# iastro-pt/gpyrn

Hardware: AMD Instinct MI355X
Metric: ELBO iterations/sec (N=4096, P=3, Q=2) (higher is better)
Workload: dtype f64; 1 GPU; BASELINE config 3: N=4096, p=3 outputs, q=2 nodes, QP nodes / SE weights, synthetic RV series (seed 0); latent_gps=8, comm_ranks=1

## Files before the change

### gpyrn_amd/_hip.py

```python
import ctypes
import os
from ctypes import POINTER, byref, c_char, c_char_p, c_double, c_int, c_int32, c_int64, c_void_p

import numpy as np

_HERE = os.path.dirname(os.path.abspath(__file__))
LIB_PATH = os.environ.get('GPRN_HIP_LIB') or os.path.join(_HERE, 'libgprn_hip.so')

GPRN_E_ARG, GPRN_E_HIP, GPRN_E_NODEV, GPRN_E_COMM, GPRN_E_NOMEM, GPRN_E_UNSUPPORTED = -1, -2, -3, -4, -5, -6
GPRN_BATCH_FORCED = 1
COV_JOINT = 1
ORDER_REFERENCE, ORDER_SEQUENTIAL = 0, 1
ELBO_REFERENCE, ELBO_BOUND = 0, 1
M_K, M_KLINV, M_SIGMA, M_BX, M_BL = 0, 1, 2, 3, 4
T_NAMES = ('fill', 'build_B', 'diag', 'panel', 'update', 'lauum', 'vec', 'update_ahead')
TILE = 128

_dp = POINTER(c_double)


class BackendUnavailable(RuntimeError):
    """libgprn_hip.so is not built, or there is no MI355X to run it on."""


# ... 13 lines not shown
    'gprn_comm_unique_id': (c_int, [POINTER(c_char)]),
    'gprn_comm_init': (c_int, [c_void_p, c_int, c_int, POINTER(c_char)]),
    'gprn_set_owners': (c_int, [c_void_p, POINTER(c_int)]),
    'gprn_comm_barrier_max': (c_int, [c_void_p, _dp]),
    'gprn_set_kernel': (c_int, [c_void_p, c_int, POINTER(c_int32), c_int, _dp, c_int, c_int]),
    'gprn_upload_K': (c_int, [c_void_p, c_int, _dp]),
    'gprn_set_y_resid': (c_int, [c_void_p, _dp]),
    'gprn_set_jitters': (c_int, [c_void_p, _dp]),
    'gprn_factor_priors': (c_int, [c_void_p]),
    'gprn_set_muvar': (c_int, [c_void_p, _dp, _dp]),
    'gprn_get_muvar': (c_int, [c_void_p, _dp, _dp]),
    'gprn_sweep': (c_int, [c_void_p, c_int, c_int, _dp, _dp]),
    'gprn_predict': (c_int, [c_void_p, c_int, _dp, _dp, _dp]),
    'gprn_predict_upload': (c_int, [c_void_p, c_int, c_int, _dp, _dp, _dp]),
    'gprn_predict_cov': (c_int, [c_void_p, c_int, _dp, c_int, _dp, _dp, _dp]),
    'gprn_predict_draws': (c_int, [c_void_p, c_int, _dp, c_int, _dp, _dp, _dp, _dp]),
    'gprn_predict_upload_kss': (c_int, [c_void_p, c_int, c_int, _dp]),
    'gprn_get_scalars': (c_int, [c_void_p, _dp]),
    'gprn_keep_sigma': (c_int, [c_void_p, c_int]),
    'gprn_get_matrix': (c_int, [c_void_p, c_int, c_int, _dp]),
    'gprn_get_logdet_K': (c_int, [c_void_p, _dp]),
    'gprn_profile_enable': (c_int, [c_void_p, c_int]),
    'gprn_profile_read': (c_int, [c_void_p, _dp, POINTER(c_int64), c_int]),
    'gprn_test_gemm': (c_int, [c_void_p, c_int, c_int, c_int, c_int, c_int, c_int, _dp, _dp, _dp]),
    'gprn_comm_allreduce_sum': (c_int, [c_void_p, _dp, c_int]),
    'gprn_test_factor_invert': (c_int, [c_void_p, c_int, c_int, _dp, _dp, _dp]),
    'gprn_test_lauum': (c_int, [c_void_p, c_int, _dp, _dp]),
    'gprn_test_gemm_rate': (c_int, [c_void_p, c_int, c_int, c_int, c_int, c_int, _dp]),
    'gprn_test_fill_rate': (c_int, [c_void_p, c_int, _dp]),
    'gprn_test_mfma_peak': (c_int, [c_void_p, c_int, c_int, _dp]),
    'gprn_test_tile_launch': (c_int, [c_void_p, c_int, c_int, _dp, c_int, POINTER(c_int64), c_int, c_int, c_int, _dp, c_int,
                              c_int]),
    'gprn_test_tile_step': (c_int, [c_void_p, c_int, _dp, c_int, c_int, c_int, c_int, POINTER(c_int64)]),
    'gprn_set_option': (c_int, [c_void_p, c_char_p, c_int, POINTER(c_int)]),
    'gprn_elbocalc_batch': (c_int, [c_void_p, c_int, _dp, c_int, _dp, _dp, _dp, _dp, c_int, _dp, POINTER(c_int), POINTER(c_int),
                            POINTER(c_int), _dp, _dp]),
    'gprn_elbocalc_batch_grad': (c_int, [c_void_p, c_int, _dp, c_int, _dp, _dp, _dp, _dp, c_int, c_int, _dp, POINTER(c_int),
                                 POINTER(c_int), POINTER(c_int), _dp, _dp, _dp]),
    'gprn_predict_batch': (c_int, [c_void_p, c_int, _dp, c_int, _dp, _dp, _dp, c_int, _dp, _dp, _dp, _dp, _dp, POINTER(c_int)]),
    'gprn_test_predict_fill': (c_int, [c_void_p, c_int, c_int, _dp, c_int, _dp, c_int, c_int, c_int, _dp, _dp, _dp, _dp]),
    'gprn_elbocalc': (c_int, [c_void_p, c_int, _dp, _dp, _dp, _dp, c_int, _dp, c_int, POINTER(c_int), POINTER(c_int),
                      POINTER(c_int), _dp, _dp]),
    'gprn_expected_loglike': (c_int, [c_void_p, _dp]),
    'gprn_prior_terms': (c_int, [c_void_p, c_int, _dp, _dp, _dp]),
    'gprn_grad_matrices': (c_int, [c_void_p, c_int, _dp, _dp]),
    'gprn_grad_kernel': (c_int, [c_void_p, c_int, _dp, _dp]),
    'gprn_grad_elbo': (c_int, [c_void_p, _dp, c_int]),
    'gprn_grad_matrix': (c_int, [c_void_p, c_int, _dp]),
    'gprn_eval_kernel': (c_int, [c_void_p, POINTER(c_int32), c_int, _dp, c_int, c_double, _dp]),
    'gprn_eval_kernel_grad': (c_int, [c_void_p, POINTER(c_int32), c_int, _dp, c_int, _dp]),
    'gprn_sample_prior': (c_int, [c_void_p, POINTER(c_int32), c_int, _dp, c_int, c_double, c_int, _dp, _dp]),
}

_lib = None


def load_library():
    global _lib
    if _lib is not None:
        return _lib
    if not os.path.exists(LIB_PATH):
        raise BackendUnavailable(
            f'{LIB_PATH} is missing: build it with `python -c "import __graft_entry__ as g; '
            f'g.build()"` (or make -C gpyrn_amd/csrc)')
    try:
        lib = ctypes.CDLL(LIB_PATH)
# ... 357 lines not shown
            raise ValueError('tstar is empty')
        jt = None
        if outputs:
            if jitters is None:
                raise ValueError('predict_batch: the output pair needs the jitters')
            jt = _f64(jitters)
            if jt.size != B * self.p:
                raise ValueError(f'jitters must be (B, p) = ({B}, {self.p}), got {jt.shape}')
        ns = ts.size
        lm = np.empty((B, self.G, ns)) if latent else None
        lv = np.empty((B, self.G, ns)) if latent else None
        om = np.empty((B, self.p, ns)) if outputs else None
        ov = np.empty((B, self.p, ns)) if outputs else None
        info = np.zeros(B, dtype=np.int32)
        opt = lambda a: None if a is None else _ptr(a)
        rc = self._lib.gprn_predict_batch(self._h, B, _ptr(kp), kp.shape[1], _ptr(m0), _ptr(v0), opt(jt), ns, _ptr(ts),
                                          opt(lm), opt(lv), opt(om), opt(ov), info.ctypes.data_as(POINTER(c_int)))
        if rc == GPRN_E_UNSUPPORTED:
            return None
        self._check(rc, 'predict_batch')
        return lm, lv, om, ov, info.astype(int)

    def test_predict_fill(self, kernel_params, var, eval_index, gp, tstar, batched):
        kp = _f64(np.atleast_2d(kernel_params))
        B = kp.shape[0]
        v0 = _f64(np.reshape(var, (B, (self.p + 1) * self.q * self.N)))
        ts = _f64(np.ravel(tstar))
        K, Ks, kss = np.empty((self.N, self.N)), np.empty((ts.size, self.N)), np.empty(ts.size)
        self._check(self._lib.gprn_test_predict_fill(self._h, int(bool(batched)), B, _ptr(kp), kp.shape[1], _ptr(v0),
                                                     int(eval_index), int(gp), ts.size, _ptr(ts), _ptr(K), _ptr(Ks), _ptr(kss)),
                    'test_predict_fill')
        return K, Ks, kss

    def option(self, name, value=-1):
        old = c_int(0)
        self._check(self._lib.gprn_set_option(self._h, name.encode(), int(value), byref(old)), 'set_option')
        return old.value

    def profile_enable(self, families=T_NAMES):
        mask = 0
        for f in families or ():
            mask |= 1 << T_NAMES.index(f)
        self._check(self._lib.gprn_profile_enable(self._h, mask), 'profile_enable')

    def profile_read(self, reset=True):
        ms = np.zeros(len(T_NAMES))
        n = np.zeros(len(T_NAMES), dtype=np.int64)
        self._check(self._lib.gprn_profile_read(self._h, _ptr(ms), n.ctypes.data_as(POINTER(c_int64)),
                                                int(bool(reset))), 'profile_read')
        return {k: (float(ms[i]), int(n[i])) for i, k in enumerate(T_NAMES)}

    def test_gemm(self, A, B, C, a_mode, b_mode, c_mode):
        A, B = _f64(A), _f64(B)
        C = _f64(C).copy()
        M, K = A.shape
        K2, N = B.shape
        assert K == K2 and C.shape == (M, N)
        self._check(self._lib.gprn_test_gemm(self._h, M, N, K, a_mode, b_mode, c_mode,
                                             _ptr(A), _ptr(B), _ptr(C)), 'test_gemm')
        return C

    def test_factor_invert(self, A):
        A = _f64(A)
        if A.ndim == 2:
            A = A[None]
        batch, n, _ = A.shape
# ... 49 lines not shown
```

### gpyrn_amd/csrc/api_sweep.hip

```cpp
#include "api_internal.h"

static int factor_priors_impl(gprn_ctx* c);

extern "C" int gprn_factor_priors(gprn_ctx* c)
{
    DeviceLock lock_(c);
    WatchScope watch_(c, "gprn_factor_priors");
    if (!c || !c->N) return bad(c, "factor_priors: call set_data first");
    HIP_TRY(c, hipSetDevice(c->device));
    if (c->owner.empty()) return bad(c, "factor_priors: call set_owners first");
    c->grad_ready = false;
    int pre = GPRN_OK;
    for (int g = 0; g < c->G && !pre; ++g)
        if (!c->kspec[g].set) pre = bad(c, "factor_priors: a latent GP has no kernel");
    if ((pre = agree_to_start(c, pre, "factor_priors"))) return pre;
    return with_event_fallback(c, "factor_priors", [&](bool) { return factor_priors_impl(c); }, true);
}

static int ensure_small_sweep_tabs(gprn_ctx* c)
{
    if (c->small_sweep_ready) return GPRN_OK;
    std::vector<double*> ktab(c->q, nullptr);
    for (int j = 1; j < c->q && c->elbo_form == GPRN_ELBO_REFERENCE; ++j) {
        if (!c->Kinv[j]) return bad(c, "small path: K_j^-1 of a node is missing (no set-up yet?)");
// ... 158 lines not shown
        const Phase setup = problem_phase(c, c->tab_setup, c->d_slotgp_setup, nb, 0, c->d_info);
        TRY(factor_invert(c, setup, true));
        TRY(vec_logdet(c, setup, BUF_B, c->d_logdetK));
        HIP_TRY(c, hipStreamSynchronize(c->stream)); watch_progress(c);
        TRY(check_info(c, c->d_info, gps, &first_info));
        for (int s = 0; s < nb; ++s) {
            const int g = gps[s];
            if (g >= c->q || !need_inv[g]) continue;
            if (!c->Kinv[g]) TRY(dev_alloc(c, &c->Kinv[g], nn));
            std::vector<double*> one((size_t)c->nslot * GPRN_NBUF, nullptr);
            one[BUF_B] = c->Kinv[g];
            one[BUF_X] = rows[s * GPRN_NBUF + BUF_X];
            HIP_TRY(c, hipStreamSynchronize(c->stream)); watch_progress(c);
            TRY(upload_table(c, c->tab_setup, one));
            TRY(lauum_lower(c, problem_phase(c, c->tab_setup, nullptr, 1, 0, nullptr)));
            HIP_TRY(c, hipStreamSynchronize(c->stream)); watch_progress(c);
            TRY(upload_table(c, c->tab_setup, rows));
        }
        HIP_TRY(c, hipStreamSynchronize(c->stream)); watch_progress(c);
    }
    {
        std::vector<double> h(c->G);
        HIP_TRY(c, hipMemcpy(h.data(), c->d_logdetK, c->G * sizeof(double), hipMemcpyDeviceToHost));
        for (int g = 0; g < c->G; ++g) if (c->owner[g] != c->rank) h[g] = 0.0;
        HIP_TRY(c, hipMemcpy(c->d_logdetK, h.data(), c->G * sizeof(double), hipMemcpyHostToDevice));
        if (comm_active(c)) TRY(comm_allreduce(c, c->d_logdetK, c->G, false));
        HIP_TRY(c, hipStreamSynchronize(c->stream)); watch_progress(c);
    }
    TRY(factor_check_waits(c));
    c->factored = true;
    return first_info;
}

static int overlap_mask(const gprn_ctx* c) { return c->overlap_opt >= 0 ? c->overlap_opt : 31; }

static Phase sweep_phase(const gprn_ctx* c, bool weights)
{
    return problem_phase(c, weights ? c->tab_weight : c->tab_node, weights ? c->d_slotgp_weight : c->d_slotgp_node,
                         (int)(weights ? c->loc_weights : c->loc_nodes).size(), weights ? (int)c->loc_nodes.size() : 0,
                         c->d_info + (weights ? 2 : 1) * (size_t)c->nslot);
}

static int small_sweep(gprn_ctx* c, const double* mu_in, const double* var_in, double* mu_out, double* var_out,
                       double* out4, double* scal, const SmallLoop* loop)
{
    c->d_scal = scal;
    const int* done = loop ? loop->ctl : nullptr;
    TRY(ensure_small_sweep_tabs(c));
    TRY(small_phase(c, sweep_phase(c, false), false, scal, mu_in, var_in, mu_out, var_out, done));
    TRY(order_small(c, sweep_phase(c, false), false, mu_in, var_in, mu_out, var_out, done));
    TRY(mask_rows(c, sweep_phase(c, false), false, mu_out, var_out, done));
    TRY(small_phase(c, sweep_phase(c, true), true, scal, mu_in, var_in, mu_out, var_out, done));
    TRY(order_small(c, sweep_phase(c, true), true, mu_in, var_in, mu_out, var_out, done));
    TRY(mask_rows(c, sweep_phase(c, true), true, mu_out, var_out, done));
    return small_tail(c, out4, scal, mu_out, var_out, loop);
}

int phase_core(gprn_ctx* c, const Phase& ph, bool weights, double* scal, std::function<int()>& chain_started)
{
    const size_t o = (size_t)ph.slot0 * ph.ld;
    TRY(order_snapshot(c, ph));
    TRY(vec_prep(c, ph, weights));
    const int overlap = overlap_mask(c);
    FactorHooks h;
    h.build_B = true;
    h.ft_s = (overlap & 1) ? c->d_s + o : nullptr;
    if (overlap & 2) {
        h.rows_final = [c, &ph, o](int r0, int r1, hipStream_t st) -> int {
            TRY(vec_lower_matvec(c, ph, BUF_X, c->d_z + o, ph.ld, 0, c->d_u + o, st, r0 * GPRN_TILE, (r1 - r0) * GPRN_TILE));
            return vec_colops_partial(c, ph, st, r0, r1 - r0);
        };
    }
    h.chain_started.swap(chain_started);
    const int rc_f = factor_invert(c, ph, false, &h);
    chain_started.swap(h.chain_started);
    TRY(rc_f);
    TRY(vec_lower_matvec(c, ph, BUF_X, c->d_z + o, ph.ld, 0, c->d_u + o, nullptr, h.rows_done * GPRN_TILE, -1));
    TRY(vec_colops_partial(c, ph, nullptr, h.rows_done, -1));
    if (overlap & 8) TRY(vec_reduce_finalize(c, ph, scal, true));
    else {
        TRY(vec_colops_reduce(c, ph));
        TRY(vec_logdet(c, ph, BUF_B, scal));
        TRY(vec_finalize(c, ph, scal, false));
    }
    TRY(order_refresh(c, ph, weights));
    return mask_rows(c, ph, weights, c->d_mu, c->d_var, nullptr);
}

static int mu_k_mu(gprn_ctx* c, bool weights, double* out, hipStream_t stream = nullptr)
{
    const Phase ph = sweep_phase(c, weights);
    if (!ph.nslots) return GPRN_OK;
    double* a = c->d_u + (size_t)ph.slot0 * ph.ld;
    TRY(vec_lower_matvec(c, ph, BUF_KLINV, c->d_mu, c->N, c->elbo_form == GPRN_ELBO_BOUND ? 2 : 1, a, stream));
    return vec_dot_self(c, ph, a, out, stream);
}

struct NodeSide {
    std::function<int()> work;
    bool q1 = false;
    bool term_done = false;
};

static int run_phase(gprn_ctx* c, bool weights, double* scal, std::function<int()>& handed, NodeSide* nodes)
{
    const Phase ph = sweep_phase(c, weights);
    const std::vector<int>& gps = weights ? c->loc_weights : c->loc_nodes;
    const int ns = ph.nslots;
    const size_t o = (size_t)ph.slot0 * ph.ld;
    if (ns) {
        TRY(phase_core(c, ph, weights, scal, handed));
        const int overlap = overlap_mask(c);
// ... 473 lines not shown
```

### gpyrn_amd/csrc/factor.hip

```cpp
#include "gprn_internal.h"
#include "tile_mma.h"
#include "diag_tile.h"
#include "vecops.h"

#include <math.h>
#include <stdlib.h>

#include <algorithm>
#include <functional>

template <bool ARGS, bool ACC>
__global__ __launch_bounds__(256) __attribute__((amdgpu_waves_per_eu(1, 1)))
void k_diag_block(double* const* __restrict__ ptrs, PtrArgs pa, int ld, int kblk, int* __restrict__ info,
                  unsigned* sig_slot, unsigned sig_value, const unsigned* wait_flag, unsigned wait_value,
                  unsigned* wait_timed_out, int nph)
{
    __shared__ __attribute__((aligned(16))) double lds[ACC ? DIAG_LDS_DOUBLES_ACC : DIAG_LDS_DOUBLES];
    if (pa.stamps && blockIdx.x == 0 && threadIdx.x == 0) pa.stamps[0] = __builtin_amdgcn_s_memrealtime();
    await_flag(wait_flag, wait_value, wait_timed_out);
    if (pa.stamps && blockIdx.x == 0 && threadIdx.x == 0) pa.stamps[1] = __builtin_amdgcn_s_memrealtime();
    const int slot = blockIdx.x;
    const size_t off = ((size_t)kblk * GPRN_TILE) * ld + (size_t)kblk * GPRN_TILE;
    double* const Bm = ARGS ? pa.p[slot][0] : ptrs[(size_t)slot * GPRN_NBUF + BUF_B];
    double* const Xm = ARGS ? pa.p[slot][1] : ptrs[(size_t)slot * GPRN_NBUF + BUF_X];
// ... 379 lines not shown
            HIP_TRY(c, raise(s1, J, F_PANEL));
            if (rest_J >= 0) HIP_TRY(c, await(s1, rest_J, sr ? F_RESTA : F_REST));
            if (next_J >= 0) { HIP_TRY(c, await(s1, next_J, F_NEXT)); next_J = -1; }
        }
        const double* const ft_s = (o.k0 == 0 && ft_fused) ? h.ft_s : nullptr;
        if (o.k1 < T) side_stamp(o.k1, 6);
        if ((rc = tiles(o.first0, o.nfirst, s1, shape_upd(o.nfirst), GPRN_T_PANEL, nosig, noaw, TG_NEXT, ft_s))) return rc;
        if (o.k1 < T) side_stamp(o.k1, 7);
        if (use_flags && folds_sync(o.k1)) pending_up = slot(J, F_FIRST) + 1;
        else HIP_TRY(c, raise(s1, J, F_FIRST));
        if (o.nfirst > 0) first_J = J;
        if (use_flags && sr && rest_J >= 0) {
            FlagOps ops = {{nullptr, nullptr}, {slot(J, F_PANEL) + 1, slot(rest_J, F_RESTA) + 1, nullptr, nullptr}};
            if ((rc = flag_multi(sn, ops))) return rc;
        } else {
            HIP_TRY(c, await(sn, J, F_PANEL));
            if (sr && rest_J >= 0) HIP_TRY(c, await(sn, rest_J, F_RESTA));
        }
        if ((rc = tiles(o.next0, o.nnext, sn, shape_upd(o.nnext), GPRN_T_PANEL, nosig, noaw, TG_NEXT, ft_s))) return rc;
        HIP_TRY(c, raise(sn, J, F_NEXT));
        if (o.nnext > 0) next_J = J;
        if (o.nrest) {
            if (sr) {
                HIP_TRY(c, await(s2, J, F_PANEL));
                if ((rc = tiles(o.rest0, o.nrestA, s2, TS_64x64, GPRN_T_UPDATE_AHEAD, nosig, noaw, TG_AHEAD, ft_s))) return rc;
                const bool resta_by_bulk = use_flags && o.nrest > o.nrestA;
                if (!resta_by_bulk) HIP_TRY(c, raise(s2, J, F_RESTA));
                if ((rc = tiles(o.rest0 + o.nrestA, o.nrest - o.nrestA, s2, TS_64x64, GPRN_T_UPDATE, nosig, noaw, TG_BULK, ft_s,
                                resta_by_bulk ? slot(J, F_RESTA) + 1 : nullptr))) return rc;
            } else if ((rc = tiles(o.rest0, o.nrest, s2, TS_64x64, GPRN_T_UPDATE, nosig, noaw, TG_BULK, ft_s))) return rc;
            HIP_TRY(c, raise(s2, J, F_REST));
            rest_J = J;
        }
        if (h.rows_final) {
            if (!(o.nrest && sr) && sn != s2) HIP_TRY(c, await(s2, J, F_PANEL));
            if ((rc = h.rows_final(o.k0, o.k1, s2))) return rc;
            h.rows_done = o.k1;
            tail_on_s2 = true;
        }
        return GPRN_OK;
    };

    for (size_t J = 0; J < c->outers[set].size(); ++J) {
        const gprn_ctx::OuterRange& o = c->outers[set][J];
        for (int k = o.k0; k < o.k1; ++k) {
            const gprn_ctx::StepRange& s = c->steps[set][k];
            if (pending_outer >= 0 && s.npanel_l == 0 && (rc = do_outer(pending_outer))) return rc;
            if ((rc = launch_diag(c, ph, k, acc, s0, in_kernel(k, F_DIAG), noaw))) return rc;
            if (!use_flags) HIP_TRY(c, raise(s0, k, F_DIAG));
            if (use_flags && k == 0 && h.chain_started) {
                HIP_TRY(c, await(s2, 0, F_DIAG));
                std::function<int()> f;
                f.swap(h.chain_started);
                if ((rc = f())) return rc;
            }
            if (s.npanel_l == 0) {
                if ((rc = flush_inner())) return rc;
                if (k > 0 && may_poll(2 * s.npanel * (size_t)nbatch)) {
                    if ((rc = tiles(s.panel0, s.npanel, s0, TS_128x64_ATRI, GPRN_T_PANEL, nosig, in_kernel_wait(k - 1, F_INNER), TG_PANEL))) return rc;
                    continue;
                }
                if (k > 0 && use_flags) { if ((rc = flag_sync(s0, nullptr, slot(k - 1, F_INNER) + 1))) return rc; }
                else if (k > 0) HIP_TRY(c, await(s0, k - 1, F_INNER));
                if ((rc = tiles(s.panel0, s.npanel, s0, TS_128x64_ATRI, GPRN_T_PANEL, nosig, noaw, TG_PANEL))) return rc;
                continue;
            }
            const bool spin = use_flags && k > 0 && nbatch <= 2;
// ... 27 lines not shown
                Await aw_d = noaw;
                if (fold_sync) {
                    if (inner_k >= 0 && !withheld(F_INNER)) up = slot(inner_k, F_INNER) + 1;
                    inner_k = -1;
                    up2 = pending_up;
                    pending_up = nullptr;
                    aw_d = in_kernel_wait(k, F_DIAG);
                }
                if ((rc = launch_panel(c, c->d_tasks + s.panel0 + 1, s.npanel_l - 1, s.npanel - s.npanel_l, ph.ptrs,
                                       nbatch, ph.ld, acc, s1, x_part_then(k), aw_d, up, epoch, up2))) return rc;
            } else {
                if ((rc = tiles(s.panel0 + 1, s.npanel_l - 1, s1, TS_64x128_BTRI, GPRN_T_PANEL, nosig, noaw, TG_PANEL))) return rc;
                if ((rc = tiles(s.panel0 + s.npanel_l, s.npanel - s.npanel_l, s1, TS_128x64_ATRI, GPRN_T_PANEL, nosig, noaw, TG_PANEL))) return rc;
                HIP_TRY(c, await(s1, k, F_MINIL));
            }
            side_stamp(k, 2);
            const size_t ncrit = s.ncol1 > 0 ? s.ncol1 - 1 : 0;
            if (use_flags && ncrit > 0 && next_J >= 0 && nbatch <= 2) {
                const bool skip = withheld(F_INNER);
                if ((rc = tiles(s.upd0 + 1, ncrit, s1, TS_64x64, GPRN_T_PANEL, skip ? nosig : in_kernel(k, F_INNER)))) return rc;
                side_stamp(k, 3);
                HIP_TRY(c, await(s1, next_J, F_NEXT));
                next_J = -1;
                side_stamp(k, 4);
                if ((rc = tiles(s.upd0 + 1 + ncrit, s.nupd - 1 - ncrit, s1, shape_upd(s.nupd - 1 - ncrit)))) return rc;
                side_stamp(k, 5);
            } else {
                if (next_J >= 0) { HIP_TRY(c, await(s1, next_J, F_NEXT)); next_J = -1; }
                side_stamp(k, 4);
                if ((rc = tiles(s.upd0 + 1, s.nupd - 1, s1, shape_upd(s.nupd - 1)))) return rc;
                side_stamp(k, 5);
                if (use_flags) inner_k = k;
                else HIP_TRY(c, raise(s1, k, F_INNER));
            }
        }
        if ((rc = flush_inner())) return rc;
        if (o.nfirst + o.nnext + o.nrest == 0) continue;
        pending_outer = (int)J;
    }
    if (pending_outer >= 0 && (rc = do_outer(pending_outer))) return rc;
    if (pending_up) { HIP_TRY(c, hipStreamWriteValue32(s1, pending_up, epoch, 0)); pending_up = nullptr; }
    if (tail_on_s2) HIP_TRY(c, raise(s2, 0, F_TAIL));
    if (use_flags) {
        FlagOps ops = {{nullptr, nullptr}, {nullptr, nullptr, nullptr, nullptr}};
        int nw = 0;
        if (first_J >= 0) ops.wait[nw++] = slot(first_J, F_FIRST) + 1;
        if (next_J >= 0) ops.wait[nw++] = slot(next_J, F_NEXT) + 1;
        if (rest_J >= 0) ops.wait[nw++] = slot(rest_J, F_REST) + 1;
        if (tail_on_s2) ops.wait[nw++] = slot(0, F_TAIL) + 1;
        return nw ? flag_multi(s0, ops) : GPRN_OK;
    }
    if (first_J >= 0) HIP_TRY(c, await(s0, first_J, F_FIRST));
    if (next_J >= 0) HIP_TRY(c, await(s0, next_J, F_NEXT));
    if (rest_J >= 0) HIP_TRY(c, await(s0, rest_J, F_REST));
    if (tail_on_s2) HIP_TRY(c, await(s0, 0, F_TAIL));
    return GPRN_OK;
}

int factor_check_waits(gprn_ctx* c)
{
    if (c->d_step_stamps && c->step_stamps_n > 0) {
        const int T = c->step_stamps_T, nph = std::min(c->step_stamps_n, 8);
        std::vector<unsigned long long> h((size_t)8 * T * 9), side;
        if (c->d_side_stamps) {
            side.resize((size_t)T * 8);
            if (hipMemcpy(side.data(), c->d_side_stamps, side.size() * sizeof(side[0]), hipMemcpyDeviceToHost) != hipSuccess) side.clear();
// ... 106 lines not shown
```

### gpyrn_amd/csrc/gprn_internal.h

```cpp
#pragma once
#include <hip/hip_runtime.h>
#include <stdint.h>
#include <algorithm>
#include <chrono>
#include <functional>
#include <string>
#include <map>
#include <mutex>
#include <vector>

#include "../../include/gprn_hip.h"
#include "batch_layout.h"

#define GPRN_TILE 128
#define GPRN_KC 16
#define GPRN_NBUF 4
#define GPRN_OUTER 4
#define GPRN_OUTER_SMALL 16
#define GPRN_LAT_MAX 32
#define GPRN_FEW_TASKS 4000
#ifndef GPRN_WIDE_CHAIN
#define GPRN_WIDE_CHAIN 48
#endif
#define GPRN_XCD_CHUNK_LOG2 4
// ... 321 lines not shown

__device__ __forceinline__ void await_flag(const unsigned* flag, unsigned value, unsigned* timed_out)
{
    if (!flag) return;
    if (threadIdx.x == 0) spin_until(flag, value, timed_out);
    __syncthreads();
}

__device__ __forceinline__ void signal_done(unsigned* slot, unsigned value, const unsigned* then_wait,
                                            unsigned then_value, unsigned* timed_out)
{
    if (!slot) return;
    asm volatile("s_waitcnt vmcnt(0)" ::: "memory");
    __syncthreads();
    if (threadIdx.x == 0) {
        if (value) {
            __builtin_amdgcn_fence(__ATOMIC_RELEASE, "agent");
            asm volatile("s_waitcnt vmcnt(0)" ::: "memory");
        }
        const unsigned total = gridDim.x * gridDim.y * gridDim.z;
        if (atomicAdd(slot, 1u) + 1 == total) {
            atomicExch(slot, 0u);
            if (value) __hip_atomic_store(slot + 1, value, __ATOMIC_RELEASE, __HIP_MEMORY_SCOPE_SYSTEM);
            if (then_wait) spin_until(then_wait, then_value, timed_out);
        }
    }
}
#endif
struct FactorHooks {
    bool build_B = false;
    const double* ft_s = nullptr;
    std::function<int(int r0, int r1, hipStream_t stream)> rows_final;
    int rows_done = 0;
    std::function<int()> chain_started;
};
int factor_invert(gprn_ctx* c, const Phase& ph, bool prior = false, FactorHooks* hooks = nullptr);
int lauum_lower(gprn_ctx* c, const Phase& ph, hipStream_t stream = nullptr);
int ensure_tasks(gprn_ctx* c, int T);
#define GPRN_E_WAIT_TIMEOUT (-100)
int factor_check_waits(gprn_ctx* c);
int factor_use_flags(gprn_ctx* c);
bool small_applies(const gprn_ctx* c);
int small_phase(gprn_ctx* c, const Phase& ph, bool weights, double* scal, const double* mu_in, const double* var_in,
                double* mu_out, double* var_out, const int* done = nullptr);
struct SmallLoop { int* ctl; double *hist, *last3; int sweep, hist_at, max_iter; };
int small_tail(gprn_ctx* c, double* out4, double* scal, const double* mu, const double* var, const SmallLoop* loop = nullptr);
int small_prior(gprn_ctx* c, double** d_tab, const int* d_job_gp, double** d_kinv_out, int njobs, int* d_info);
struct BatchIo {
    int n; const double* kparams; int n_kpar; const double *y_resid, *jitters, *mu, *var; int max_iter;
    double* elbo; int *iters, *conv, *info; double *mu_out, *var_out;
    int p; size_t state, yv;
    int flags;
    double* grad_out;
    BatchIo slice(int e0, int ne) const
    {
        return BatchIo{ne, kparams + (size_t)e0 * n_kpar, n_kpar, y_resid + e0 * yv, jitters + (size_t)e0 * p, mu + e0 * state,
                       var + e0 * state, max_iter, elbo + e0, iters + e0, conv + e0, info + e0,
                       mu_out ? mu_out + e0 * state : nullptr, var_out ? var_out + e0 * state : nullptr, p, state, yv,
                       flags, grad_out ? grad_out + (size_t)e0 * n_kpar : nullptr};
    }
};
struct GradBatchIn {
    int N, ld, T, q, G;
    const double* t;
    int n = 0;
    std::vector<double*> rows;
// ... 105 lines not shown
```

### gpyrn_amd/csrc/vecops.h

```cpp
#pragma once
#include "gprn_internal.h"

int vec_prep(gprn_ctx* c, const Phase& ph, bool weights);
int vec_build_B(gprn_ctx* c, const Phase& ph, hipStream_t stream = nullptr, int part = 0, int outer = 0);
int vec_logdet(gprn_ctx* c, const Phase& ph, int buf, double* out);
int vec_lower_matvec(gprn_ctx* c, const Phase& ph, int buf, const double* vin, size_t vstride, int vin_by_gp,
                     double* out, hipStream_t stream = nullptr, int row0 = 0, int nrows = -1);
int vec_colops(gprn_ctx* c, const Phase& ph);
int vec_colops_partial(gprn_ctx* c, const Phase& ph, hipStream_t stream, int ch0, int nch);
int vec_colops_reduce(gprn_ctx* c, const Phase& ph);
int vec_reduce_finalize(gprn_ctx* c, const Phase& ph, double* scal, bool with_logdet);
int vec_finalize(gprn_ctx* c, const Phase& ph, double* scal, bool with_logdet = false);
int vec_q1(gprn_ctx* c, const double* Kinv_j, const double* Binv_k, const double* s_k,
           double* scratch, double* out_scalar, hipStream_t stream);
int vec_dot_self(gprn_ctx* c, const Phase& ph, const double* a, double* out, hipStream_t stream = nullptr);
int vec_elbo(gprn_ctx* c, double* out4, const double* scal, double* part, hipStream_t stream = nullptr);
#define GPRN_ELBO_PART_DOUBLES (3 * 32)
int vec_elbo_evals(gprn_ctx* c, const EvalMap& ev, const int* d_evals, int n, double* out4, const double* scal, double* part,
                   hipStream_t stream = nullptr);
int vec_q1_evals(gprn_ctx* c, const Phase& ph, const double* Kinv_slab, int n_eval, double* scratch, double* q1,
                 hipStream_t stream = nullptr);
int vec_sigma(gprn_ctx* c, const double* Binv, const double* s, double* out);
int vec_pred_rows(gprn_ctx* c, const Phase& ph, int ns, int ns_pad, const double* sol, const double* kss,
                  double* mean, double* var);
int vec_predict_outputs(gprn_ctx* c, int n_eval, int ns, size_t pitch, const double* lat_mean, const double* lat_var,
                        const double* jit, double* out_mean, double* out_var);
int vec_axpy_matrix(gprn_ctx* c, const double* src, double* dst, int N);
int vec_symmetrize(gprn_ctx* c, double* M);
int vec_grad_contract(gprn_ctx* c, int kid, const double* par, const double* Kinv, const double* P, const double* m,
                      double* a_scratch, double* part_scratch, double* out4);
int vec_symv(gprn_ctx* c, const double* M, const double* v, double* out);
```

### gpyrn_amd/csrc/vecops.hip

```cpp
#include "gprn_internal.h"
#include "vecops.h"
#include "grad_elem.h"

#include <math.h>

#include <algorithm>

typedef double v2d __attribute__((ext_vector_type(2)));

__device__ __forceinline__ double wave_sum(double v)
{
#pragma unroll
    for (int o = 32; o > 0; o >>= 1) v += __shfl_down(v, o, 64);
    return v;
}

__device__ __forceinline__ double block_sum(double v, double* sh )
{
    v = wave_sum(v);
    const int lane = threadIdx.x & 63, w = threadIdx.x >> 6;
    __syncthreads();
    if (lane == 0) sh[w] = v;
    __syncthreads();
    double r = 0.0;
// ... 142 lines not shown
    __shared__ double sh[4];
    const int slot = blockIdx.x;
    const double* M = ptrs[(size_t)slot * GPRN_NBUF + buf];
    double acc = 0.0;
    for (int n = threadIdx.x; n < N; n += 256) acc += log(M[(size_t)n * ld + n]);
    acc = block_sum(acc, sh);
    if (threadIdx.x == 0) out[ev_of(ev, slot) * out_stride + slot_gp[slot]] = 2.0 * acc;
}

__global__ __launch_bounds__(256)
void k_lower_matvec(double* const* __restrict__ ptrs, int buf, int N, int ld,
                    const double* __restrict__ vin, size_t vstride, int vin_by_gp,
                    const int* __restrict__ slot_gp, double* __restrict__ out, int row0, EvalMap ev, int p, int q)
{
    const int slot = blockIdx.y;
    const int i = row0 + blockIdx.x * 4 + (threadIdx.x >> 6), lane = threadIdx.x & 63;
    if (i >= ld) return;
    const double* M = ptrs[(size_t)slot * GPRN_NBUF + buf] + (size_t)i * ld;
    const double* v = vin + (vin_by_gp ? ev_of(ev, slot) * ev.state +
                                         (size_t)(vin_by_gp == 2 ? own_state_row(slot_gp[slot], p, q) : slot_gp[slot]) * vstride
                                       : (size_t)slot * vstride);
    double acc = 0.0;
    if (i < N) {
        for (int c = 2 * lane; c <= i; c += 128) {
            const v2d mv = *reinterpret_cast<const v2d*>(M + c);
            acc += mv.x * v[c];
            if (c + 1 <= i) acc += mv.y * v[c + 1];
        }
    }
    acc = wave_sum(acc);
    if (lane == 0) out[(size_t)slot * ld + i] = acc;
}

__global__ __launch_bounds__(256)
void k_colops_partial(double* const* __restrict__ ptrs, int ld, int T,
                      const double* __restrict__ u, double* __restrict__ part, int ch0)
{
    __shared__ double shs[4][64], sht[4][64];
    const int c0 = blockIdx.x * 64, ch = ch0 + blockIdx.y, slot = blockIdx.z;
    if (ch < (c0 >> 7)) return;
    const double* X = ptrs[(size_t)slot * GPRN_NBUF + BUF_X];
    const double* uv = u + (size_t)slot * ld;
    const int cl = threadIdx.x & 63, rl = threadIdx.x >> 6;
    double cs = 0.0, ct = 0.0;
    for (int r0 = ch * GPRN_TILE + rl; r0 < (ch + 1) * GPRN_TILE; r0 += 32) {
        double x[8], w[8];
#pragma unroll
        for (int k = 0; k < 8; ++k) {
            x[k] = X[(size_t)(r0 + 4 * k) * ld + c0 + cl];
            w[k] = uv[r0 + 4 * k];
        }
#pragma unroll
        for (int k = 0; k < 8; ++k) {
            cs += x[k] * x[k];
            ct += x[k] * w[k];
        }
    }
    shs[rl][cl] = cs;
    sht[rl][cl] = ct;
    __syncthreads();
    if (rl == 0) {
        const size_t o = (((size_t)slot * T + ch) * 2) * ld + c0 + cl;
        part[o] = (shs[0][cl] + shs[1][cl]) + (shs[2][cl] + shs[3][cl]);
        part[o + ld] = (sht[0][cl] + sht[1][cl]) + (sht[2][cl] + sht[3][cl]);
    }
}

__global__ __launch_bounds__(256)
void k_colops_reduce(int ld, int T, const double* __restrict__ part,
                     double* __restrict__ cs, double* __restrict__ ct)
{
    const int slot = blockIdx.y, c = blockIdx.x * 256 + threadIdx.x;
    if (c >= ld) return;
    double a = 0.0, b = 0.0;
    for (int ch = c >> 7; ch < T; ++ch) {
        const size_t o = (((size_t)slot * T + ch) * 2) * ld + c;
        a += part[o];
        b += part[o + ld];
    }
    cs[(size_t)slot * ld + c] = a;
    ct[(size_t)slot * ld + c] = b;
}

template <bool MASKED>
__global__ __launch_bounds__(256)
void k_finalize(const int* __restrict__ slot_gp, int N, int ld, int p, int q,
                const double* __restrict__ d, const double* __restrict__ s,
                const double* __restrict__ z, const double* __restrict__ cs, const double* __restrict__ ct,
                double* __restrict__ mu, double* __restrict__ var, double* __restrict__ trBinv,
                double* const* __restrict__ ptrs, double* __restrict__ logdetB, EvalMap ev)
{
    __shared__ double sh[4];
    const int slot = blockIdx.x, gp = slot_gp[slot];
    const size_t eb = ev_of(ev, slot);
    mu += eb * ev.state; var += eb * ev.state; trBinv += eb * ev.scal; logdetB += eb * ev.scal;
    size_t row;
    if (gp < q) row = gp;
// ... 13 lines not shown
    if (threadIdx.x == 0) trBinv[gp] = tr;
    if (Lm) {
        ld_acc = block_sum(ld_acc, sh);
        if (threadIdx.x == 0) logdetB[gp] = 2.0 * ld_acc;
    }
}

template <bool FENCED, bool MASKED>
__global__ __launch_bounds__(256)
void k_reduce_finalize(const int* __restrict__ slot_gp, int N, int ld, int T, int p, int q,
                       const double* __restrict__ part, const double* __restrict__ d, const double* __restrict__ s,
                       const double* __restrict__ z, double* __restrict__ cs, double* __restrict__ ct,
                       double* __restrict__ mu, double* __restrict__ var, double* __restrict__ trBinv,
                       double* const* __restrict__ ptrs, double* __restrict__ logdetB,
                       double* __restrict__ terms , unsigned* __restrict__ tickets , EvalMap ev)
{
    __shared__ double sh[4];
    __shared__ unsigned last;
    const int slot = blockIdx.y, gp = slot_gp[slot], n = blockIdx.x * 256 + threadIdx.x;
    const size_t eb = ev_of(ev, slot);
    mu += eb * ev.state; var += eb * ev.state; trBinv += eb * ev.scal; logdetB += eb * ev.scal;
    size_t row;
    if (gp < q) row = gp;
    else { const int kk = gp - q, j = kk / p, i = kk % p; row = (size_t)(1 + i) * q + j; }
    const double* Lm = ptrs ? ptrs[(size_t)slot * GPRN_NBUF + BUF_B] : nullptr;
    double* const tt = terms + (size_t)slot * 2 * ld;
    if (n < ld) {
        double a = 0.0, b = 0.0;
        for (int ch = n >> 7; ch < T; ++ch) {
            const size_t o = (((size_t)slot * T + ch) * 2) * ld + n;
            a += part[o];
            b += part[o + ld];
        }
        const size_t o = (size_t)slot * ld + n;
        cs[o] = a;
        ct[o] = b;
        if (n < N) {
            mu[row * N + n] = (z[o] - b) / s[o];
            var[row * N + n] = (1.0 - a) / d[o];
            if (MASKED && d[o] == 0.0) { mu[row * N + n] = 0.0; var[row * N + n] = 0.0; }
            __hip_atomic_store(tt + n, a, __ATOMIC_RELAXED, __HIP_MEMORY_SCOPE_AGENT);
            if (Lm) __hip_atomic_store(tt + ld + n, log(Lm[(size_t)n * ld + n]), __ATOMIC_RELAXED, __HIP_MEMORY_SCOPE_AGENT);
        }
    }
    constexpr bool fenced = FENCED || !GPRN_RELAXED_HANDOVER;
    if (fenced) __builtin_amdgcn_fence(__ATOMIC_RELEASE, "agent");
    asm volatile("s_waitcnt vmcnt(0)" ::: "memory");
    __syncthreads();
    if (threadIdx.x == 0) {
        const unsigned got = fenced ? __hip_atomic_fetch_add(tickets + slot, 1u, __ATOMIC_ACQ_REL, __HIP_MEMORY_SCOPE_AGENT)
                                    : __hip_atomic_fetch_add(tickets + slot, 1u, __ATOMIC_RELAXED, __HIP_MEMORY_SCOPE_AGENT);
        last = got + 1 == gridDim.x ? 1u : 0u;
    }
    __syncthreads();
    if (!last) return;
    if (fenced) __builtin_amdgcn_fence(__ATOMIC_ACQUIRE, "agent");
    double tr = 0.0, ld_acc = 0.0;
    for (int m = threadIdx.x; m < N; m += 256) {
        tr += __hip_atomic_load(tt + m, __ATOMIC_RELAXED, __HIP_MEMORY_SCOPE_AGENT);
        if (Lm) ld_acc += __hip_atomic_load(tt + ld + m, __ATOMIC_RELAXED, __HIP_MEMORY_SCOPE_AGENT);
    }
    tr = block_sum(tr, sh);
    if (threadIdx.x == 0) { trBinv[gp] = tr; atomicExch(tickets + slot, 0u); }
    if (Lm) {
        ld_acc = block_sum(ld_acc, sh);
        if (threadIdx.x == 0) logdetB[gp] = 2.0 * ld_acc;
// ... 189 lines not shown
                       (double* const*)ph.ptrs, ph.ld, ph.T, c->d_u + o, c->d_part + po, ch0);
    LAUNCH_END(c);
}

int vec_colops_reduce(gprn_ctx* c, const Phase& ph)
{
    if (!ph.nslots) return GPRN_OK;
    prof_begin(c, GPRN_T_VEC);
    const size_t o = (size_t)ph.slot0 * ph.ld, po = (size_t)ph.slot0 * ph.T * 2 * ph.ld;
    hipLaunchKernelGGL(k_colops_reduce, dim3((ph.ld + 255) / 256, ph.nslots), dim3(256), 0,
                       c->stream, ph.ld, ph.T, c->d_part + po, c->d_cs + o, c->d_ct + o);
    LAUNCH_END(c);
}

int vec_colops(gprn_ctx* c, const Phase& ph)
{
    int rc = vec_colops_partial(c, ph, nullptr, 0, -1);
    return rc ? rc : vec_colops_reduce(c, ph);
}

int vec_finalize(gprn_ctx* c, const Phase& ph, double* scal, bool with_logdet)
{
    if (!ph.nslots) return GPRN_OK;
    prof_begin(c, GPRN_T_VEC);
    const size_t o = (size_t)ph.slot0 * ph.ld;
#define GO_FIN(M) hipLaunchKernelGGL(k_finalize<M>, dim3(ph.nslots), dim3(256), 0, c->stream, ph.slot_gp, ph.N, ph.ld, \
                       c->p, c->q, c->d_d + o, c->d_s + o, c->d_z + o, c->d_cs + o, c->d_ct + o, c->d_mu, c->d_var, \
                       scal + c->G, with_logdet ? (double* const*)ph.ptrs : (double* const*)nullptr, scal, ph.ev)
    if (c->d_mask) GO_FIN(true); else GO_FIN(false);
#undef GO_FIN
    LAUNCH_END(c);
}

int vec_reduce_finalize(gprn_ctx* c, const Phase& ph, double* scal, bool with_logdet)
{
    if (!ph.nslots) return GPRN_OK;
    prof_begin(c, GPRN_T_VEC);
    const size_t o = (size_t)ph.slot0 * ph.ld, po = (size_t)ph.slot0 * ph.T * 2 * ph.ld;
#define GO_RF(F, M) hipLaunchKernelGGL((k_reduce_finalize<F, M>), dim3((ph.ld + 255) / 256, ph.nslots), dim3(256), 0, c->stream, ph.slot_gp, ph.N, \
                       ph.ld, ph.T, c->p, c->q, c->d_part + po, c->d_d + o, c->d_s + o, c->d_z + o, c->d_cs + o, c->d_ct + o, c->d_mu, \
                       c->d_var, scal + c->G, with_logdet ? (double* const*)ph.ptrs : (double* const*)nullptr, scal, \
                       c->d_fin_terms + (size_t)ph.slot0 * 2 * ph.ld, c->d_fin_tickets + ph.slot0, ph.ev)
    if (c->d_mask) { if (c->fenced_finalize) GO_RF(true, true); else GO_RF(false, true); }
    else           { if (c->fenced_finalize) GO_RF(true, false); else GO_RF(false, false); }
#undef GO_RF
    LAUNCH_END(c);
}

int vec_q1(gprn_ctx* c, const double* Kinv_j, const double* Binv_k, const double* s_k,
           double* scratch, double* out_scalar, hipStream_t stream)
{
    prof_begin(c, GPRN_T_VEC, stream);
    hipLaunchKernelGGL(k_q1_rows, dim3((c->N + 3) / 4), dim3(256), 0, stream, Kinv_j, Binv_k,
                       c->N, c->ld, s_k, scratch);
    hipLaunchKernelGGL(k_sum_to, dim3(1), dim3(256), 0, stream, scratch, c->N, out_scalar);
    LAUNCH_END(c);
}

int vec_dot_self(gprn_ctx* c, const Phase& ph, const double* a, double* out, hipStream_t stream)
{
    if (!ph.nslots) return GPRN_OK;
    if (!stream) stream = c->stream;
    prof_begin(c, GPRN_T_VEC, stream);
    hipLaunchKernelGGL(k_dot_self, dim3(ph.nslots), dim3(256), 0, stream, ph.slot_gp, ph.N, ph.ld,
                       a, out, ph.ev);
    LAUNCH_END(c);
}

int vec_elbo(gprn_ctx* c, double* out4, const double* scal, double* part, hipStream_t stream)
{
    if (!stream) stream = c->stream;
    prof_begin(c, GPRN_T_VEC, stream);
    const EvalMap one{nullptr, 0, 0, 0, 0};
    const bool bound = c->elbo_form == GPRN_ELBO_BOUND;
#define GO_LL(M, B, Y, MASK) hipLaunchKernelGGL((k_loglike_partial<M, B>), dim3(ELBO_BLOCKS), dim3(256), 0, stream, c->N, c->p, c->q, \
                           c->d_mu, c->d_var, Y, c->d_variance, part, (const int*)nullptr, one, (const uint8_t*)MASK)
#define GO_EF(B) hipLaunchKernelGGL(k_elbo_final<B>, dim3(1), dim3(64), 0, stream, c->N, c->p, c->q, part, \
                       c->d_logdetK, scal, scal + c->G, scal + 2 * (size_t)c->G, scal + 3 * (size_t)c->G, out4, \
// ... 263 lines not shown
```

### include/gprn_hip.h

```cpp
#ifndef GPRN_HIP_H
#define GPRN_HIP_H

#include <stdint.h>

#ifdef __cplusplus
extern "C" {
#endif

typedef struct gprn_ctx gprn_ctx;

enum {
    GPRN_OK = 0,
    GPRN_E_ARG = -1,
    GPRN_E_HIP = -2,
    GPRN_E_NODEV = -3,
    GPRN_E_COMM = -4,
    GPRN_E_NOMEM = -5,
    GPRN_E_UNSUPPORTED = -6
};

enum {
    GPRN_K_CONSTANT = 0,
    GPRN_K_WHITENOISE = 1,
    GPRN_K_SE = 2,
// ... 112 lines not shown
                        int max_iter, double* elbo, int* iterations, int* converged, int* info,
                        double* mu_out, double* var_out);

#define GPRN_BATCH_FORCED 1
int gprn_elbocalc_batch_grad(gprn_ctx* ctx, int n_eval, const double* kernel_params, int n_kernel_params,
                             const double* y_resid, const double* jitters, const double* mu, const double* var,
                             int max_iter, int flags, double* elbo, int* iterations, int* converged, int* info,
                             double* mu_out, double* var_out, double* grad_out);

int gprn_predict_batch(gprn_ctx* ctx, int n_eval, const double* kernel_params, int n_kernel_params,
                       const double* mu, const double* var, const double* jitters, int ns, const double* tstar,
                       double* lat_mean, double* lat_var, double* out_mean, double* out_var, int* info);

int gprn_set_option(gprn_ctx* ctx, const char* name, int value, int* old);

#define GPRN_ELBO_REFERENCE 0
#define GPRN_ELBO_BOUND 1

int gprn_test_gemm(gprn_ctx* ctx, int M, int N, int K, int a_mode, int b_mode,
                   int c_mode, const double* A, const double* B, double* C);
int gprn_test_gemm_rate(gprn_ctx* ctx, int M, int N, int K, int how, int reps, double* ms);
int gprn_test_fill_rate(gprn_ctx* ctx, int reps, double* ms);
int gprn_test_factor_invert(gprn_ctx* ctx, int n, int batch, const double* A,
                            double* L, double* Linv);
int gprn_test_mfma_peak(gprn_ctx* ctx, int wg_per_cu, int iters, double* tflops);
int gprn_test_lauum(gprn_ctx* ctx, int n, const double* X, double* out);
int gprn_test_tile_launch(gprn_ctx* ctx, int ld, int nbatch, double* bufs, int ntasks, const int64_t* tasks,
                          int shape, int tag, int ldc, const double* ft_s, int ft_n, int acc);
int gprn_test_tile_step(gprn_ctx* ctx, int nbatch, double* bufs, int which, int table, int n_l, int n_x,
                        const int64_t* tasks);
int gprn_test_predict_fill(gprn_ctx* ctx, int batched, int n_eval, const double* kernel_params, int n_kernel_params,
                           const double* var, int eval, int gp, int ns, const double* tstar,
                           double* K_out, double* Ks_out, double* kss_out);

#ifdef __cplusplus
}
#endif
#endif
```

Baseline: 117.2 sweeps/s.

## Run per-row finalize eagerly during factorization and fuse last row into reduce

Adds an eager mode where the per-tile-row matvec and column-op work is issued on the side stream as soon as each row's inner update completes, instead of per panel. The last tile row's column ops are fused into the reduce-finalize kernel, saving a launch. Both are turned on by default through new bits in the overlap mask. This adds cross-stream waits and flag logic, and it declares a test entry point whose implementation is not visible.

```diff
diff --git a/gpyrn_amd/_hip.py b/gpyrn_amd/_hip.py
--- a/gpyrn_amd/_hip.py
+++ b/gpyrn_amd/_hip.py
@@ -69,6 +69,7 @@
     'gprn_test_tile_launch': (c_int, [c_void_p, c_int, c_int, _dp, c_int, POINTER(c_int64), c_int, c_int, c_int, _dp, c_int,
                               c_int]),
     'gprn_test_tile_step': (c_int, [c_void_p, c_int, _dp, c_int, c_int, c_int, c_int, POINTER(c_int64)]),
+    'gprn_test_finalize': (c_int, [c_void_p, c_int, c_int, _dp, _dp, _dp]),
     'gprn_set_option': (c_int, [c_void_p, c_char_p, c_int, POINTER(c_int)]),
     'gprn_elbocalc_batch': (c_int, [c_void_p, c_int, _dp, c_int, _dp, _dp, _dp, _dp, c_int, _dp, POINTER(c_int), POINTER(c_int),
                             POINTER(c_int), _dp, _dp]),
@@ -492,6 +493,14 @@
                     'test_predict_fill')
         return K, Ks, kss
 
+    def test_finalize(self, weights, fused):
+        ns = self.p * self.q if weights else self.q
+        ld = TILE * ((self.N + TILE - 1) // TILE)
+        cs, ct, scal = np.empty((ns, ld)), np.empty((ns, ld)), np.empty((2, self.q * (self.p + 1)))
+        self._check(self._lib.gprn_test_finalize(self._h, int(bool(weights)), int(bool(fused)), _ptr(cs), _ptr(ct), _ptr(scal)),
+                    'test_finalize')
+        return cs, ct, scal
+
     def option(self, name, value=-1):
         old = c_int(0)
         self._check(self._lib.gprn_set_option(self._h, name.encode(), int(value), byref(old)), 'set_option')
diff --git a/gpyrn_amd/csrc/api_sweep.hip b/gpyrn_amd/csrc/api_sweep.hip
--- a/gpyrn_amd/csrc/api_sweep.hip
+++ b/gpyrn_amd/csrc/api_sweep.hip
@@ -214,7 +214,7 @@
     return first_info;
 }
 
-static int overlap_mask(const gprn_ctx* c) { return c->overlap_opt >= 0 ? c->overlap_opt : 31; }
+static int overlap_mask(const gprn_ctx* c) { return c->overlap_opt >= 0 ? c->overlap_opt : 31 + 64 + 128; }
 
 static Phase sweep_phase(const gprn_ctx* c, bool weights)
 {
@@ -247,19 +247,22 @@
     FactorHooks h;
     h.build_B = true;
     h.ft_s = (overlap & 1) ? c->d_s + o : nullptr;
-    if (overlap & 2) {
+    if (overlap & (2 | 64)) {
         h.rows_final = [c, &ph, o](int r0, int r1, hipStream_t st) -> int {
             TRY(vec_lower_matvec(c, ph, BUF_X, c->d_z + o, ph.ld, 0, c->d_u + o, st, r0 * GPRN_TILE, (r1 - r0) * GPRN_TILE));
             return vec_colops_partial(c, ph, st, r0, r1 - r0);
         };
     }
+    h.rows_by_panel = (overlap & 2) != 0;
+    h.rows_eager = (overlap & 64) != 0;
     h.chain_started.swap(chain_started);
     const int rc_f = factor_invert(c, ph, false, &h);
     chain_started.swap(h.chain_started);
     TRY(rc_f);
     TRY(vec_lower_matvec(c, ph, BUF_X, c->d_z + o, ph.ld, 0, c->d_u + o, nullptr, h.rows_done * GPRN_TILE, -1));
-    TRY(vec_colops_partial(c, ph, nullptr, h.rows_done, -1));
-    if (overlap & 8) TRY(vec_reduce_finalize(c, ph, scal, true));
+    const bool fuse_last = (overlap & 8) && (overlap & 128);
+    TRY(vec_colops_partial(c, ph, nullptr, h.rows_done, fuse_last ? ph.T - 1 - h.rows_done : -1));
+    if (overlap & 8) TRY(vec_reduce_finalize(c, ph, scal, true, fuse_last));
     else {
         TRY(vec_colops_reduce(c, ph));
         TRY(vec_logdet(c, ph, BUF_B, scal));
diff --git a/gpyrn_amd/csrc/factor.hip b/gpyrn_amd/csrc/factor.hip
--- a/gpyrn_amd/csrc/factor.hip
+++ b/gpyrn_amd/csrc/factor.hip
@@ -435,7 +435,7 @@
             HIP_TRY(c, raise(s2, J, F_REST));
             rest_J = J;
         }
-        if (h.rows_final) {
+        if (h.rows_final && h.rows_by_panel) {
             if (!(o.nrest && sr) && sn != s2) HIP_TRY(c, await(s2, J, F_PANEL));
             if ((rc = h.rows_final(o.k0, o.k1, s2))) return rc;
             h.rows_done = o.k1;
@@ -529,6 +529,15 @@
                 side_stamp(k, 5);
                 if (use_flags) inner_k = k;
                 else HIP_TRY(c, raise(s1, k, F_INNER));
+            }
+            if (h.rows_final && h.rows_eager && set == 0 && o.k1 == T && k == h.rows_done) {
+                if (use_flags) {
+                    FlagOps ops = {{nullptr, nullptr}, {slot(k, F_INNER) + 1, nullptr, nullptr, nullptr}};
+                    if ((rc = flag_multi(s2, ops))) return rc;
+                } else HIP_TRY(c, await(s2, k, F_INNER));
+                if ((rc = h.rows_final(k, k + 1, s2))) return rc;
+                h.rows_done = k + 1;
+                tail_on_s2 = true;
             }
         }
         if ((rc = flush_inner())) return rc;
diff --git a/gpyrn_amd/csrc/gprn_internal.h b/gpyrn_amd/csrc/gprn_internal.h
--- a/gpyrn_amd/csrc/gprn_internal.h
+++ b/gpyrn_amd/csrc/gprn_internal.h
@@ -377,6 +377,7 @@
     const double* ft_s = nullptr;
     std::function<int(int r0, int r1, hipStream_t stream)> rows_final;
     int rows_done = 0;
+    bool rows_by_panel = true, rows_eager = false;
     std::function<int()> chain_started;
 };
 int factor_invert(gprn_ctx* c, const Phase& ph, bool prior = false, FactorHooks* hooks = nullptr);
diff --git a/gpyrn_amd/csrc/vecops.h b/gpyrn_amd/csrc/vecops.h
--- a/gpyrn_amd/csrc/vecops.h
+++ b/gpyrn_amd/csrc/vecops.h
@@ -9,7 +9,7 @@
 int vec_colops(gprn_ctx* c, const Phase& ph);
 int vec_colops_partial(gprn_ctx* c, const Phase& ph, hipStream_t stream, int ch0, int nch);
 int vec_colops_reduce(gprn_ctx* c, const Phase& ph);
-int vec_reduce_finalize(gprn_ctx* c, const Phase& ph, double* scal, bool with_logdet);
+int vec_reduce_finalize(gprn_ctx* c, const Phase& ph, double* scal, bool with_logdet, bool last_row = false);
 int vec_finalize(gprn_ctx* c, const Phase& ph, double* scal, bool with_logdet = false);
 int vec_q1(gprn_ctx* c, const double* Kinv_j, const double* Binv_k, const double* s_k,
            double* scratch, double* out_scalar, hipStream_t stream);
diff --git a/gpyrn_amd/csrc/vecops.hip b/gpyrn_amd/csrc/vecops.hip
--- a/gpyrn_amd/csrc/vecops.hip
+++ b/gpyrn_amd/csrc/vecops.hip
@@ -198,15 +198,9 @@
     if (lane == 0) out[(size_t)slot * ld + i] = acc;
 }
 
-__global__ __launch_bounds__(256)
-void k_colops_partial(double* const* __restrict__ ptrs, int ld, int T,
-                      const double* __restrict__ u, double* __restrict__ part, int ch0)
-{
-    __shared__ double shs[4][64], sht[4][64];
-    const int c0 = blockIdx.x * 64, ch = ch0 + blockIdx.y, slot = blockIdx.z;
-    if (ch < (c0 >> 7)) return;
-    const double* X = ptrs[(size_t)slot * GPRN_NBUF + BUF_X];
-    const double* uv = u + (size_t)slot * ld;
+__device__ __forceinline__ void colops_tile_row(const double* __restrict__ X, const double* __restrict__ uv, int ld, int ch,
+                                                int c0, double (*shs)[64], double (*sht)[64], double& cs_out, double& ct_out)
+{
     const int cl = threadIdx.x & 63, rl = threadIdx.x >> 6;
     double cs = 0.0, ct = 0.0;
     for (int r0 = ch * GPRN_TILE + rl; r0 < (ch + 1) * GPRN_TILE; r0 += 32) {
@@ -226,9 +220,27 @@
     sht[rl][cl] = ct;
     __syncthreads();
     if (rl == 0) {
+        cs_out = (shs[0][cl] + shs[1][cl]) + (shs[2][cl] + shs[3][cl]);
+        ct_out = (sht[0][cl] + sht[1][cl]) + (sht[2][cl] + sht[3][cl]);
+    }
+}
+
+__global__ __launch_bounds__(256)
+void k_colops_partial(double* const* __restrict__ ptrs, int ld, int T,
+                      const double* __restrict__ u, double* __restrict__ part, int ch0)
+{
+    __shared__ double shs[4][64], sht[4][64];
+    const int c0 = blockIdx.x * 64, ch = ch0 + blockIdx.y, slot = blockIdx.z;
+    if (ch < (c0 >> 7)) return;
+    const double* X = ptrs[(size_t)slot * GPRN_NBUF + BUF_X];
+    const double* uv = u + (size_t)slot * ld;
+    const int cl = threadIdx.x & 63, rl = threadIdx.x >> 6;
+    double cs = 0.0, ct = 0.0;
+    colops_tile_row(X, uv, ld, ch, c0, shs, sht, cs, ct);
+    if (rl == 0) {
         const size_t o = (((size_t)slot * T + ch) * 2) * ld + c0 + cl;
-        part[o] = (shs[0][cl] + shs[1][cl]) + (shs[2][cl] + shs[3][cl]);
-        part[o + ld] = (sht[0][cl] + sht[1][cl]) + (sht[2][cl] + sht[3][cl]);
+        part[o] = cs;
+        part[o + ld] = ct;
     }
 }
 
@@ -308,6 +320,78 @@
             a += part[o];
             b += part[o + ld];
         }
+        const size_t o = (size_t)slot * ld + n;
+        cs[o] = a;
+        ct[o] = b;
+        if (n < N) {
+            mu[row * N + n] = (z[o] - b) / s[o];
+            var[row * N + n] = (1.0 - a) / d[o];
+            if (MASKED && d[o] == 0.0) { mu[row * N + n] = 0.0; var[row * N + n] = 0.0; }
+            __hip_atomic_store(tt + n, a, __ATOMIC_RELAXED, __HIP_MEMORY_SCOPE_AGENT);
+            if (Lm) __hip_atomic_store(tt + ld + n, log(Lm[(size_t)n * ld + n]), __ATOMIC_RELAXED, __HIP_MEMORY_SCOPE_AGENT);
+        }
+    }
+    constexpr bool fenced = FENCED || !GPRN_RELAXED_HANDOVER;
+    if (fenced) __builtin_amdgcn_fence(__ATOMIC_RELEASE, "agent");
+    asm volatile("s_waitcnt vmcnt(0)" ::: "memory");
+    __syncthreads();
+    if (threadIdx.x == 0) {
+        const unsigned got = fenced ? __hip_atomic_fetch_add(tickets + slot, 1u, __ATOMIC_ACQ_REL, __HIP_MEMORY_SCOPE_AGENT)
+                                    : __hip_atomic_fetch_add(tickets + slot, 1u, __ATOMIC_RELAXED, __HIP_MEMORY_SCOPE_AGENT);
+        last = got + 1 == gridDim.x ? 1u : 0u;
+    }
+    __syncthreads();
+    if (!last) return;
+    if (fenced) __builtin_amdgcn_fence(__ATOMIC_ACQUIRE, "agent");
+    double tr = 0.0, ld_acc = 0.0;
+    for (int m = threadIdx.x; m < N; m += 256) {
+        tr += __hip_atomic_load(tt + m, __ATOMIC_RELAXED, __HIP_MEMORY_SCOPE_AGENT);
+        if (Lm) ld_acc += __hip_atomic_load(tt + ld + m, __ATOMIC_RELAXED, __HIP_MEMORY_SCOPE_AGENT);
+    }
+    tr = block_sum(tr, sh);
+    if (threadIdx.x == 0) { trBinv[gp] = tr; atomicExch(tickets + slot, 0u); }
+    if (Lm) {
+        ld_acc = block_sum(ld_acc, sh);
+        if (threadIdx.x == 0) logdetB[gp] = 2.0 * ld_acc;
+    }
+}
+
+template <bool FENCED, bool MASKED>
+__global__ __launch_bounds__(256)
+void k_rows_reduce_finalize(const int* __restrict__ slot_gp, int N, int ld, int T, int p, int q,
+                            const double* __restrict__ u, double* part, const double* __restrict__ d,
+                            const double* __restrict__ s, const double* __restrict__ z, double* __restrict__ cs,
+                            double* __restrict__ ct, double* __restrict__ mu, double* __restrict__ var,
+                            double* __restrict__ trBinv, double* const* __restrict__ ptrs, bool with_logdet,
+                            double* __restrict__ logdetB, double* __restrict__ terms ,
+                            unsigned* __restrict__ tickets , EvalMap ev)
+{
+    __shared__ double shs[4][64], sht[4][64];
+    __shared__ double sh[4];
+    __shared__ unsigned last;
+    const int slot = blockIdx.y, gp = slot_gp[slot], c0 = blockIdx.x * 64;
+    const int cl = threadIdx.x & 63, rl = threadIdx.x >> 6, n = c0 + cl;
+    const size_t eb = ev_of(ev, slot);
+    mu += eb * ev.state; var += eb * ev.state; trBinv += eb * ev.scal; logdetB += eb * ev.scal;
+    size_t row;
+    if (gp < q) row = gp;
+    else { const int kk = gp - q, j = kk / p, i = kk % p; row = (size_t)(1 + i) * q + j; }
+    const double* Lm = with_logdet ? ptrs[(size_t)slot * GPRN_NBUF + BUF_B] : nullptr;
+    double* const tt = terms + (size_t)slot * 2 * ld;
+    double ps = 0.0, pt = 0.0;
+    colops_tile_row(ptrs[(size_t)slot * GPRN_NBUF + BUF_X], u + (size_t)slot * ld, ld, T - 1, c0, shs, sht, ps, pt);
+    if (rl == 0) {
+        const size_t ol = (((size_t)slot * T + (T - 1)) * 2) * ld + n;
+        part[ol] = ps;
+        part[ol + ld] = pt;
+        double a = 0.0, b = 0.0;
+        for (int ch = n >> 7; ch < T - 1; ++ch) {
+            const size_t o = (((size_t)slot * T + ch) * 2) * ld + n;
+            a += part[o];
+            b += part[o + ld];
+        }
+        a += ps;
+        b += pt;
         const size_t o = (size_t)slot * ld + n;
         cs[o] = a;
         ct[o] = b;
@@ -563,7 +647,7 @@
     LAUNCH_END(c);
 }
 
-int vec_reduce_finalize(gprn_ctx* c, const Phase& ph, double* scal, bool with_logdet)
+int vec_reduce_finalize(gprn_ctx* c, const Phase& ph, double* scal, bool with_logdet, bool last_row)
 {
     if (!ph.nslots) return GPRN_OK;
     prof_begin(c, GPRN_T_VEC);
@@ -572,9 +656,18 @@
                        ph.ld, ph.T, c->p, c->q, c->d_part + po, c->d_d + o, c->d_s + o, c->d_z + o, c->d_cs + o, c->d_ct + o, c->d_mu, \
                        c->d_var, scal + c->G, with_logdet ? (double* const*)ph.ptrs : (double* const*)nullptr, scal, \
                        c->d_fin_terms + (size_t)ph.slot0 * 2 * ph.ld, c->d_fin_tickets + ph.slot0, ph.ev)
-    if (c->d_mask) { if (c->fenced_finalize) GO_RF(true, true); else GO_RF(false, true); }
-    else           { if (c->fenced_finalize) GO_RF(true, false); else GO_RF(false, false); }
+#define GO_RRF(F, M) hipLaunchKernelGGL((k_rows_reduce_finalize<F, M>), dim3(ph.ld / 64, ph.nslots), dim3(256), 0, c->stream, ph.slot_gp, ph.N, \
+                       ph.ld, ph.T, c->p, c->q, c->d_u + o, c->d_part + po, c->d_d + o, c->d_s + o, c->d_z + o, c->d_cs + o, c->d_ct + o, \
+                       c->d_mu, c->d_var, scal + c->G, (double* const*)ph.ptrs, with_logdet, scal, \
+                       c->d_fin_terms + (size_t)ph.slot0 * 2 * ph.ld, c->d_fin_tickets + ph.slot0, ph.ev)
+    if (last_row) {
+        if (c->d_mask) { if (c->fenced_finalize) GO_RRF(true, true); else GO_RRF(false, true); }
+        else           { if (c->fenced_finalize) GO_RRF(true, false); else GO_RRF(false, false); }
+    }
+    else if (c->d_mask) { if (c->fenced_finalize) GO_RF(true, true); else GO_RF(false, true); }
+    else                { if (c->fenced_finalize) GO_RF(true, false); else GO_RF(false, false); }
 #undef GO_RF
+#undef GO_RRF
     LAUNCH_END(c);
 }
 
diff --git a/include/gprn_hip.h b/include/gprn_hip.h
--- a/include/gprn_hip.h
+++ b/include/gprn_hip.h
@@ -168,6 +168,7 @@
 int gprn_test_predict_fill(gprn_ctx* ctx, int batched, int n_eval, const double* kernel_params, int n_kernel_params,
                            const double* var, int eval, int gp, int ns, const double* tstar,
                            double* K_out, double* Ks_out, double* kss_out);
+int gprn_test_finalize(gprn_ctx* ctx, int weights, int fused, double* cs_out, double* ct_out, double* scal_out);
 
 #ifdef __cplusplus
 }
```

Measured after the change: 117.6 sweeps/s (median of 6 runs). Within noise of the previous version (+0.3%).
